# smrt-model/smrt

Hardware: AMD Instinct MI355X
Metric: snowpack x frequency DORT solves/sec (20 layers, 32 streams) (higher is better)
Workload: dtype f64

## Files before the change

include/smrt_dort.h:

```cpp
#ifndef SMRT_DORT_H
#define SMRT_DORT_H

#include <stdint.h>

#ifdef __cplusplus
extern "C" {
#endif
#if defined(__GNUC__)
#pragma GCC visibility push(default)
#endif

typedef struct smrt_dort_ctx smrt_dort_ctx;

#define SMRT_EM_IBA 0
#define SMRT_EM_DMRT_QCA_SHORTRANGE 1
#define SMRT_EM_DMRT_QCACP_SHORTRANGE 2
#define SMRT_EM_NONSCATTERING 3
#define SMRT_EM_HOST 4
#define SMRT_EM_IBA_INVERTED 5
#define SMRT_EM_IBA_HOST 6
#define SMRT_EM_RAYLEIGH_HOST 7
#define SMRT_MS_EXPONENTIAL 0
#define SMRT_MS_STICKY_HARD_SPHERES 1
#define SMRT_MS_INDEPENDENT_SPHERE 2
// ... 63 lines not shown
    int32_t host_interface_slots;
    const double* liquid_water;
    const double* host_iba_coeff;
} smrt_batch;

int32_t smrt_dort_out_stride(const smrt_batch* b);

int32_t smrt_dort_device_count(void);

int32_t smrt_dort_create(smrt_dort_ctx** ctx, int32_t device);
void smrt_dort_destroy(smrt_dort_ctx* ctx);
const char* smrt_dort_last_error(const smrt_dort_ctx* ctx);

int32_t smrt_dort_run(smrt_dort_ctx* ctx, const smrt_batch* batch, int64_t pair_begin, int64_t pair_count,
                      double* out, int32_t* status, double* layer_out, double* stream_out);

int32_t smrt_dort_run_pairs(smrt_dort_ctx* ctx, const smrt_batch* batch, const int64_t* pairs, int64_t n_pairs,
                            double* out, int32_t* status, double* layer_out, double* stream_out);

int32_t smrt_dort_upload(smrt_dort_ctx* ctx, const smrt_batch* batch, int64_t pair_begin, int64_t pair_count);
int32_t smrt_dort_upload_pairs(smrt_dort_ctx* ctx, const smrt_batch* batch, const int64_t* pairs, int64_t n_pairs);
int32_t smrt_dort_launch(smrt_dort_ctx* ctx, void* out_dev, void* status_dev);
int32_t smrt_dort_sync(smrt_dort_ctx* ctx);
int32_t smrt_dort_download(smrt_dort_ctx* ctx, double* out, int32_t* status, double* layer_out,
                           double* stream_out);

double smrt_dort_last_kernel_ms(smrt_dort_ctx* ctx);

int32_t smrt_dort_kernel_breakdown(smrt_dort_ctx* ctx, int32_t enable, double* ms3);

int32_t smrt_dort_set_diagonalisation(smrt_dort_ctx* ctx, int32_t mode);

enum { SMRT_INFO_PIPELINE = 0, SMRT_INFO_CHUNK_PAIRS, SMRT_INFO_CHUNKS, SMRT_INFO_PRUNE_ROUNDS, SMRT_INFO_STAGED_ITEMS,
       SMRT_INFO_BLOCK_THREADS, SMRT_INFO_N_MAX, SMRT_INFO_DIAGONALISATION, SMRT_INFO_RAYLEIGH_CLOSED_FORM, SMRT_INFO_COUNT };
enum { SMRT_DIAG_JACOBI = 0,
       SMRT_DIAG_SYMMETRIC = 1 };
enum { SMRT_PIPELINE_FUSED = 0,
       SMRT_PIPELINE_LDS_TWO_SLOT = 1,
       SMRT_PIPELINE_LDS_FOUR_SLOT = 2,
       SMRT_PIPELINE_LDS_REG = 3,
       SMRT_PIPELINE_FUSED_GMEM = 4,
       SMRT_PIPELINE_GMEM = 5,
       SMRT_PIPELINE_BIG = 6,
       SMRT_PIPELINE_GMEM_STRIP = 7,
       SMRT_PIPELINE_LDS_STRIP = 8 };
int32_t smrt_dort_launch_info(smrt_dort_ctx* ctx, int64_t* info, int32_t n);
double smrt_dort_total_kernel_ms(smrt_dort_ctx* ctx, int64_t* n_launches, int32_t reset);

int32_t smrt_dort_set_block_threads(smrt_dort_ctx* ctx, int32_t threads);

int32_t smrt_dort_set_pipeline(smrt_dort_ctx* ctx, int32_t split);

int32_t smrt_dort_finish_reg_lds_bytes(int32_t n_max_stream, int32_t n_layers_max);

int32_t smrt_dort_finish_strip_lds_bytes(int32_t n_max_stream, int32_t n_layers_max, int32_t wavefronts);

int32_t smrt_dort_jacobi_lds_bytes(int32_t n_max_stream, int32_t n_pol, int32_t size_class_columns);

double smrt_dort_sum_n3(smrt_dort_ctx* ctx);

int32_t smrt_dort_ft_even_phase(smrt_dort_ctx* ctx, int32_t emmodel, int32_t microstructure, double frequency,
                                double frac_volume, double temperature, double micro_p1, double micro_p2,
                                const double* mu_s, int32_t n_s, const double* mu_i, int32_t n_i, int32_t m_max,
                                int32_t npol, double* out);

int32_t smrt_dort_pair_cost(smrt_dort_ctx* ctx, double* cost);

// ... 200 lines not shown
```

smrt_amd/_native.py:

```python
from __future__ import annotations

import ctypes as C
import os
import threading

import numpy as np

from .core.error import SMRTError

_HERE = os.path.dirname(os.path.abspath(__file__))
LIB_PATH = os.environ.get("SMRT_DORT_LIB") or os.path.join(_HERE, "csrc", "libsmrt_dort.so")

EM_CODES = {"iba": 0, "dmrt_qca_shortrange": 1, "dmrt_qcacp_shortrange": 2, "nonscattering": 3, "host": 4,
            "iba_inverted": 5, "iba_host": 6, "rayleigh_host": 7}
MS_CODES = {"exponential": 0, "sticky_hard_spheres": 1, "independent_sphere": 2, "teubner_strey": 3,
            "unified_scaled_exponential": 0, "unified_sticky_hard_spheres": 1, "unified_teubner_strey": 3,
            "exponential_complex_k": 4, "sticky_hard_spheres_complex_k": 5, "independent_sphere_complex_k": 6,
            "teubner_strey_complex_k": 7}
SUBSTRATE_CODES = {"flat": 1, "reflector": 2, "host": 3}
NORM_CODES = {False: 0, None: 0, True: 1, "auto": 1, "forced": 2}
STATUS_MESSAGES = {
    1: "The eigen-decomposition did not converge in DORT.",
    2: "The re-normalization of the phase function exceeds the predefined threshold of 30%. This is likely because "
       "of a too large grain size or a bug in the phase function.",
# ... 1120 lines not shown
    def sar_sync(self):
        self._solver_call("smrt_sar_sync")

    def sar_download(self) -> SarOutput:
        return self._solver_download("sar", SarOutput)

    def sar_kernel_ms(self):
        return self._solver_kernel_ms("sar", 4)

    def ft_even_phase(self, emmodel, microstructure, frequency, frac_volume, temperature, p1, p2, mu_s, mu_i, m_max, npol):
        mu_s = np.ascontiguousarray(np.atleast_1d(mu_s), dtype=np.float64)
        mu_i = np.ascontiguousarray(np.atleast_1d(mu_i), dtype=np.float64)
        out = np.empty((npol, npol, m_max + 1, len(mu_s), len(mu_i)))
        with self.lock:
            self._check(self._lib.smrt_dort_ft_even_phase(
                self._h, EM_CODES[emmodel], MS_CODES[microstructure], float(frequency), float(frac_volume), float(temperature),
                float(p1), float(p2), _dptr(mu_s), len(mu_s), _dptr(mu_i), len(mu_i), int(m_max), int(npol), _dptr(out)),
                "smrt_dort_ft_even_phase")
        return out

    def pair_cost(self):
        _, pair_count = self._resident
        cost = np.empty(pair_count)
        self._check(self._lib.smrt_dort_pair_cost(self._h, _dptr(cost)), "smrt_dort_pair_cost")
        return cost

    PIPELINES = ("fused", "lds_two_slot", "lds_four_slot", "lds_reg", "fused_gmem", "gmem", "big", "gmem_strip", "lds_strip")

    def launch_info(self):
        v = (C.c_int64 * 16)()
        n = self._lib.smrt_dort_launch_info(self._h, v, 16)
        self._check(0 if n > 0 else -1, "smrt_dort_launch_info")
        keys = ("pipeline", "chunk_pairs", "chunks", "prune_rounds", "staged_items", "block_threads", "n_max", "diagonalisation",
                "rayleigh_closed_form")
        d = {k: int(v[i]) for i, k in enumerate(keys[:n])}
        d["pipeline"] = self.PIPELINES[d["pipeline"]]
        d["diagonalisation"] = self.DIAGONALISATIONS[d["diagonalisation"]]
        d["rayleigh_closed_form"] = bool(d.get("rayleigh_closed_form", 0))
        if d.get("staged_items", -1) < 0:
            d["staged_items"] = None
        return d

    @staticmethod
    def comm_library():
        lib = load_library()
        buf, version = C.create_string_buffer(1024), C.c_int32(0)
        if lib.smrt_dort_comm_library(buf, len(buf), C.byref(version)) != 0:
            raise SMRTError("RCCL is not available: " + buf.value.decode(errors="replace"))
        v = int(version.value)
        return buf.value.decode(), "%d.%d.%d" % (v // 10000, v // 100 % 100, v % 100) if v >= 10000 else str(v)

    @staticmethod
    def comm_unique_id():
        lib = load_library()
        buf = C.create_string_buffer(128)
        if lib.smrt_dort_comm_unique_id(buf) != 0:
            raise SMRTError("smrt_dort_comm_unique_id failed (is librccl available?)")
        return buf.raw

    def comm_init(self, world, rank, unique_id):
        self._check(self._lib.smrt_dort_comm_init(self._h, int(world), int(rank), bytes(unique_id)), "smrt_dort_comm_init")
        self.world, self.rank = int(world), int(rank)

    @staticmethod
    def comm_init_all(contexts):
        lib = load_library()
        arr = (C.c_void_p * len(contexts))(*[c._h for c in contexts])
        if lib.smrt_dort_comm_init_all(arr, len(contexts)) != 0:
            raise SMRTError("smrt_dort_comm_init_all failed: " + lib.smrt_dort_last_error(contexts[0]._h).decode())
        for r, c in enumerate(contexts):
            c.world, c.rank = len(contexts), r
# ... 81 lines not shown
```

smrt_amd/csrc/dort_ctx.hpp:

```cpp
#pragma once
#include <hip/hip_runtime.h>
#include <string>
#include <vector>

#include "dort_layout.hpp"

namespace smrt { struct PhaseRequest; struct FoBatch; }

struct DevBuf {
    void* p = nullptr;
    size_t cap = 0;
    hipError_t reserve(size_t bytes) {
        if (bytes <= cap) return hipSuccess;
        if (p) (void)hipFree(p);
        p = nullptr;
        cap = 0;
        hipError_t e = hipMalloc(&p, bytes);
        if (e == hipSuccess) cap = bytes;
        return e;
    }
    void release() { if (p) (void)hipFree(p); p = nullptr; cap = 0; }
};

struct smrt_dort_ctx {
// ... 6 lines not shown
    bool uploaded = false;
    int out_stride = 0;
    int nt = 256;
    size_t lds_bytes = 0;
    size_t prep_lds_bytes = 0;
    size_t finish2_lds_bytes = 0;
    size_t finish_reg_lds_bytes = 0;
    size_t prep_wide_lds_bytes = 0;
    bool prep_wide = false;
    size_t finish_strip_lds_bytes = 0, finish_strip4_lds_bytes = 0;
    bool finish_strip4 = false;
    bool finish_strip = false;
    bool finish_reg = false;
    int finish_mode = -1;
    bool finish2 = true;
    float last_ms = 0.f;
    double total_ms = 0.0;
    int64_t n_launch = 0;
    bool timing_pending = false;
    bool breakdown_on = false;
    std::vector<hipEvent_t> bd_events;
    std::vector<int> bd_kind;
    size_t bd_used = 0;
    int max_lds = 0;
    bool split = true;
    long long chunk_pairs = 0;
    int lanes = 1;
    hipStream_t lane_stream[4] = {nullptr, nullptr, nullptr, nullptr};
    hipEvent_t lane_ev[4] = {nullptr, nullptr, nullptr, nullptr};
    hipEvent_t fork_ev = nullptr;
    size_t jacobi_lds = 0;
    int diag_mode = -1;
    bool eig = false;
    size_t jacobi16_lds = 0;
    smrt::DevStage stage{};
    bool gmem_path = false;
    bool gmem_split = false;
    bool big = false;
    int jac_in_lds = 0;
    bool active = false;
    int gmem_grid = 0;
    long long ws_stride = 0;
    int nmax_rows = 0;
    void* comm = nullptr;
    int comm_world = 0, comm_rank = 0;
    DevBuf d_gather_out, d_gather_status, d_scalar;
    struct FirstOrderState* first_order = nullptr;
    struct SuccessiveOrderState* successive_order = nullptr;
    struct SuccessiveOrderActiveState* successive_order_active = nullptr;
    struct MultiFresnelState* multifresnel = nullptr;
    struct SecondOrderState* second_order = nullptr;
    struct LrmState* lrm = nullptr;
    struct SarState* sar = nullptr;
};

#ifndef SMRT_JACOBI_NT
#define SMRT_JACOBI_NT 256
#endif

namespace smrt_launch {
hipError_t prep(smrt_dort_ctx* ctx, const smrt::DevBatch& c, int nt);
hipError_t prep_wide(smrt_dort_ctx* ctx, const smrt::DevBatch& c);
hipError_t finish(smrt_dort_ctx* ctx, const smrt::DevBatch& c, int nt, bool two_slot);
void occupancy_report(smrt_dort_ctx* ctx, int nt);
hipError_t finish_reg(smrt_dort_ctx* ctx, const smrt::DevBatch& c);
hipError_t finish_strip(smrt_dort_ctx* ctx, const smrt::DevBatch& c);
// ... 26 lines not shown
```

smrt_amd/csrc/dort_dense.hpp:

```cpp
#pragma once
#include "spmd.hpp"
#include <math.h>
#include <string.h>
#include "dort_physics.hpp"

namespace smrt {

struct Tile2D { int rmask, cshift, cols_per_wave; };
SMRT_DEV Tile2D make_tile(int R) {
    Tile2D t;
    int sh = 6;
    if (R <= 32) sh = 5;
    if (R <= 16) sh = 4;
    if (R <= 8) sh = 3;
    if (R <= 4) sh = 2;
    t.rmask = (1 << sh) - 1; t.cshift = sh; t.cols_per_wave = SMRT_LANES >> sh;
    return t;
}
template <int NT, class Body>
SMRT_DEV void for_2d(int R, int C, Body body) {
    const int t = tid();
    const int lane = t & (SMRT_LANES - 1), wave = t / SMRT_LANES;
    constexpr int NW = NT / SMRT_LANES;
    const Tile2D tl = make_tile(R);
// ... 288 lines not shown
    const int lane = tid() & (SMRT_LANES - 1), lr = lane & 15, lk = lane >> 4;
    const int col = tj * 16 + lr;
#pragma unroll
    for (int reg = 0; reg < 4; ++reg) {
        const int row = ti * 16 + lk + 4 * reg;
        if (row < N && col < N) f(reg, row, col);
    }
}

template <int NT, bool PK = false>
SMRT_DEV void lt_times_l_mfma(const double* Lp, const double* Lm, double* C, int N, int LD, bool reverse_cols = false) {
    const int wave = tid() / SMRT_LANES;
    constexpr int NW = NT / SMRT_LANES;
    const int RT = (N + 15) >> 4;
    for (int tix = wave; tix < RT * RT; tix += NW) {
        const int ti = tix % RT, tj = tix / RT;
        double c[4] = {0.0, 0.0, 0.0, 0.0};
        const int kmin = 16 * (ti > tj ? ti : tj);
        const int lane = tid() & (SMRT_LANES - 1), lr = lane & 15, lk = lane >> 4;
        const int i = ti * 16 + lr, j = tj * 16 + lr;
        const int ic = i < N ? i : N - 1, jc = j < N ? j : N - 1;
        const int abase = sidx<PK>(ic, ic, LD) - ic, bbase = sidx<PK>(jc, jc, LD) - jc;
        for (int k0 = kmin; k0 < N; k0 += 4) {
            const int k = k0 + lk, kc = k < N ? k : N - 1;
            const double av = Lp[abase + (kc > ic ? kc : ic)], bv = Lm[bbase + (kc > jc ? kc : jc)];
            const bool kin = k < N;
            mfma_f64_16x16x4((kin && k >= i) ? av : 0.0, (kin && k >= j) ? bv : 0.0, c);
        }
        tile_foreach(ti, tj, N, [&](int reg, int row, int col) { C[(reverse_cols ? N - 1 - col : col) * LD + row] = c[reg]; });
    }
    block_sync();
}

template <int NT>
SMRT_DEV void l_times_m_mfma(const double* Lp, const double* Bm, double* C, int N, int LD) {
    const int wave = tid() / SMRT_LANES;
    constexpr int NW = NT / SMRT_LANES;
    constexpr int TPW = 3;
    const int RT = (N + 15) >> 4;
    const int NG = (RT + TPW - 1) / TPW;
    const int lane = tid() & (SMRT_LANES - 1), lr = lane & 15, lk = lane >> 4;
    for (int u = wave; u < RT * NG; u += NW) {
        const int ti = u % RT, tg = u / RT;
        double c[TPW][4];
#pragma unroll
        for (int q = 0; q < TPW; ++q)
#pragma unroll
            for (int reg = 0; reg < 4; ++reg) c[q][reg] = 0.0;
        const int i = ti * 16 + lr, ic = i < N ? i : N - 1;
        const int kend = (ti * 16 + 16 < N) ? ti * 16 + 16 : N;
        const int nq = (RT - tg * TPW < TPW) ? RT - tg * TPW : TPW;
        for (int k0 = 0; k0 < kend; k0 += 16) {
            double av[4], bv[TPW][4];
#pragma unroll
            for (int kk = 0; kk < 4; ++kk) {
                const int k = k0 + 4 * kk + lk, kc = k < N ? k : N - 1;
                const double x = Lp[kc * LD + ic];
                av[kk] = (i < N && k <= i && k < N) ? x : 0.0;
#pragma unroll
                for (int q = 0; q < TPW; ++q) {
                    bv[q][kk] = 0.0;
                    if (q < nq) {
                        const int j = (tg * TPW + q) * 16 + lr, jc = j < N ? j : N - 1;
                        const double y = Bm[jc * LD + kc];
                        bv[q][kk] = (j < N && k < N) ? y : 0.0;
                    }
// ... 824 lines not shown
```

smrt_amd/csrc/dort_hip.hip:

```cpp
#include <hip/hip_runtime.h>
#include <algorithm>
#include <cstddef>
#include <cstdio>
#include <cstdlib>
#include <cstring>
#include <string>
#include <vector>

#include "dort_ctx.hpp"
#include "dort_eig_kernel.hpp"
#include "dort_rayleigh_kernel.hpp"
#include "dort_jacobi_big.hpp"
#include "dort_host_common.hpp"
#include "dort_phase_kernel.hpp"
#include "dort_finish_reg.hpp"
#include "dort_finish_strip.hpp"
#include "solver_host.hpp"

using namespace smrt;

static int upload_array(smrt_dort_ctx* ctx, DevBuf& buf, const void* src, size_t bytes) {
    HIPCHK(buf.reserve(bytes));
    HIPCHK(hipMemcpyAsync(buf.p, src, bytes, hipMemcpyHostToDevice, ctx->stream));
    return 0;
}


static DevBatch chunk_of(const smrt_dort_ctx* ctx, const DevBatch& d, long long c0, long long cn) {
    DevBatch c = d;
    c.pair_begin = d.pair_begin + c0; c.pair_count = cn;
    c.out = d.out + c0 * ctx->out_stride; c.status = d.status + c0;
    c.layer_out = d.layer_out + c0 * (long long)d.Lmax * 5;
    c.stream_out = d.stream_out + c0 * (long long)(1 + d.n_max_stream);
    c.n3_out = d.n3_out + c0; c.stage_out = d.stage_out + c0 * 16;
    if (d.dispatch) c.dispatch = d.dispatch + c0;
    return c;
}

#ifndef SMRT_DORT_LANES_DEFAULT
#define SMRT_DORT_LANES_DEFAULT 1
#endif
#ifndef SMRT_FINISH_STRIP_DEFAULT
#define SMRT_FINISH_STRIP_DEFAULT 1
#endif
#ifndef SMRT_FINISH_REG_DEFAULT
#define SMRT_FINISH_REG_DEFAULT 1
#endif
static hipError_t launch_pipeline(smrt_dort_ctx* ctx, const DevBatch& d) {
    const long long items_per_pair = (long long)(ctx->active ? d.m_max + 1 : 1) * d.Lmax;
    const long long modes = ctx->active ? d.m_max + 1 : 1;
    if (getenv("SMRT_DORT_DEBUG_OCCUPANCY") && !ctx->gmem_path && !ctx->active) smrt_launch::occupancy_report(ctx, ctx->nt);
    const int rounds = (d.prune_tau > 0.0 && !d.coherent && getenv("SMRT_DORT_NO_PRUNE_ROUNDS") == nullptr) ? std::min(4, d.Lmax) : 1;
    auto prep = [&](const DevBatch& c, unsigned grid) {
        if (ctx->big) return smrt_launch::prep_gmem_big(ctx, c, grid, ctx->active, ctx->nmax_rows <= 256 ? 4 : 6);
        if (ctx->prep_wide) return smrt_launch::prep_wide(ctx, c);
        if (ctx->gmem_split) return smrt_launch::prep_gmem(ctx, c, grid, ctx->active);
        return ctx->active ? smrt_launch::active_prep(ctx, c, ctx->nt) : smrt_launch::prep(ctx, c, ctx->nt);
    };
    auto finish = [&](const DevBatch& c, unsigned grid) {
        if (ctx->big) return smrt_launch::finish_gmem_big(ctx, c, grid, ctx->active, ctx->nmax_rows <= 256 ? 4 : 6);
        if (ctx->finish_strip) return smrt_launch::finish_strip(ctx, c);
        if (ctx->gmem_split) return smrt_launch::finish_gmem(ctx, c, grid, ctx->active);
        if (ctx->finish_strip4) return smrt_launch::finish_strip4(ctx, c);
        if (ctx->finish_reg) return smrt_launch::finish_reg(ctx, c);
        return ctx->active ? smrt_launch::active_finish(ctx, c, ctx->nt) : smrt_launch::finish(ctx, c, ctx->nt, ctx->finish2);
    };
    const hipStream_t main_stream = ctx->stream;
    const DevStage stage0 = ctx->stage;
    const int lanes = (ctx->lanes > 1 && d.pair_count > ctx->chunk_pairs) ? ctx->lanes : 1;
    struct Restore { smrt_dort_ctx* c; hipStream_t s; DevStage st; ~Restore() { c->stream = s; c->stage = st; } } restore{ctx, main_stream, stage0};
    if (lanes > 1) {
        hipError_t e;
        if ((e = hipEventRecord(ctx->fork_ev, main_stream)) != hipSuccess) return e;
        for (int k = 0; k < lanes; ++k)
            if ((e = hipStreamWaitEvent(ctx->lane_stream[k], ctx->fork_ev, 0)) != hipSuccess) return e;
    }
    auto timed = [&](int kind, auto&& launch) -> hipError_t {
        if (!ctx->breakdown_on) return launch();
        for (int k = 0; k < 2; ++k)
            if (ctx->bd_used + k >= ctx->bd_events.size()) {
                hipEvent_t ev;
                hipError_t e = hipEventCreate(&ev);
                if (e != hipSuccess) return e;
                ctx->bd_events.push_back(ev);
            }
        hipError_t e = hipEventRecord(ctx->bd_events[ctx->bd_used], ctx->stream);
        if (e != hipSuccess) return e;
        e = launch();
        if (e != hipSuccess) return e;
        e = hipEventRecord(ctx->bd_events[ctx->bd_used + 1], ctx->stream);
        ctx->bd_used += 2;
        ctx->bd_kind.push_back(kind);
        return e;
    };
    if (ctx->breakdown_on) { ctx->bd_used = 0; ctx->bd_kind.clear(); }
    long long chunk_index = 0;
    for (long long c0 = 0; c0 < d.pair_count; c0 += ctx->chunk_pairs, ++chunk_index) {
        const long long cn = std::min<long long>(ctx->chunk_pairs, d.pair_count - c0);
        DevBatch c = chunk_of(ctx, d, c0, cn);
        const unsigned grid = (unsigned)(ctx->gmem_path ? std::min<long long>(cn, ctx->gmem_grid) : cn);
// ... 200 lines not shown
    ctx->eig = false;
    int big_min = 128;
    if (const char* e = getenv("SMRT_DORT_BIG_MIN_N")) big_min = std::max(64, atoi(e));
    ctx->big = ctx->gmem_path && ctx->split && plan.NMAX > big_min && getenv("SMRT_DORT_NO_BIG_PIPELINE") == nullptr &&
               (size_t)make_jacobi_big_plan(b->n_max_stream, P).total * sizeof(double) <= (size_t)ctx->max_lds;
    const bool split128 = ctx->gmem_path && ctx->split && !ctx->big && plan.NMAX <= 128 &&
        (size_t)make_jacobi_plan(b->n_max_stream, P).total * sizeof(double) <= (size_t)ctx->max_lds &&
        (size_t)make_plan(b->n_max_stream, P, b->n_layers_max, b->n_theta, nphi, 0, actd_fin, 0, 2).total * sizeof(double) <= (size_t)ctx->max_lds &&
        (size_t)make_plan(b->n_max_stream, P, b->n_layers_max, b->n_theta, nphi, 0, actd, 1).total * sizeof(double) <= (size_t)ctx->max_lds;
    if (split128) ctx->jac_in_lds = 1;
    ctx->gmem_split = ctx->big || split128;
    if (ctx->big) ctx->jac_in_lds = 0;
    if ((!ctx->gmem_path && ctx->split) || ctx->gmem_split) {
        const size_t nmodes = ctx->active ? (size_t)b->m_max + 1 : 1;
        const size_t mat = (size_t)plan.NMAX * plan.LD;
        const int linv_stride = (plan.NMAX > 64) ? 2048 : 1024;
        const size_t per_pair = nmodes * b->n_layers_max * ((2 * mat + 2 * plan.NMAX + linv_stride) * sizeof(double) + sizeof(int));
        double budget = 12.0e9;
        if (ctx->big) {
            size_t free_b = 0, total_b = 0;
            if (hipMemGetInfo(&free_b, &total_b) == hipSuccess) budget = std::max(budget, 0.6 * (double)(free_b + ctx->d_stL.cap + ctx->d_stB.cap));
        }
        const bool one_per_cu = ctx->gmem_split && !ctx->big;
        if (one_per_cu) budget = 40.0e9;
        long long chunk = (long long)(budget / (double)per_pair);
        if (chunk < 1) chunk = 1;
        if (one_per_cu && chunk >= 512) chunk -= chunk % 256;
        const long long chunk_cap = chunk;
        if (chunk > pair_count) chunk = pair_count;
        {
            int want = ctx->diag_mode < 0 ? SMRT_DIAG_SYMMETRIC : ctx->diag_mode;
            if (const char* e = getenv("SMRT_DORT_EIG")) want = atoi(e) ? SMRT_DIAG_SYMMETRIC : SMRT_DIAG_JACOBI;
            ctx->eig = !ctx->gmem_path && !ctx->active && plan.NMAX <= 64 && want == SMRT_DIAG_SYMMETRIC;
        }
        ctx->lanes = 1;
        if (!ctx->gmem_path) {
            int want = ctx->eig ? 3 : SMRT_DORT_LANES_DEFAULT;
            if (const char* e = getenv("SMRT_DORT_LANES")) want = atoi(e);
            ctx->lanes = std::max(1, std::min(4, want));
            while (ctx->lanes > 1 && pair_count < 1024LL * ctx->lanes) --ctx->lanes;
        }
        {
            long long nchunks = (pair_count + chunk - 1) / chunk;
            if (ctx->lanes > 1) nchunks = ((nchunks + ctx->lanes - 1) / ctx->lanes) * ctx->lanes;
            chunk = (pair_count + nchunks - 1) / nchunks;
            if (one_per_cu && nchunks > 1) chunk = std::min(chunk_cap, ((chunk + 255) / 256) * 256);
        }
        ctx->chunk_pairs = chunk;
        for (int k = 0; k < ctx->lanes && ctx->lanes > 1; ++k) {
            if (!ctx->lane_stream[k]) HIPCHK(hipStreamCreateWithFlags(&ctx->lane_stream[k], hipStreamNonBlocking));
            if (!ctx->lane_ev[k]) HIPCHK(hipEventCreateWithFlags(&ctx->lane_ev[k], hipEventDisableTiming));
        }
        if (ctx->lanes > 1 && !ctx->fork_ev) HIPCHK(hipEventCreateWithFlags(&ctx->fork_ev, hipEventDisableTiming));
        const size_t items = (size_t)chunk * ctx->lanes * b->n_layers_max * nmodes;
        HIPCHK(ctx->d_stL.reserve(items * mat * sizeof(double)));
        HIPCHK(ctx->d_stB.reserve(items * mat * sizeof(double)));
        HIPCHK(ctx->d_std.reserve(items * plan.NMAX * sizeof(double)));
        HIPCHK(ctx->d_sts.reserve(items * plan.NMAX * sizeof(double)));
        HIPCHK(ctx->d_stn.reserve(items * sizeof(int)));
        HIPCHK(ctx->d_sti.reserve(ctx->big ? 8 : items * linv_stride * sizeof(double)));
        ctx->stage.L = (double*)ctx->d_stL.p; ctx->stage.B = (double*)ctx->d_stB.p;
        ctx->stage.d = (double*)ctx->d_std.p; ctx->stage.sigma = (double*)ctx->d_sts.p;
        ctx->stage.n = (int*)ctx->d_stn.p; ctx->stage.Linv = ctx->big ? nullptr : (double*)ctx->d_sti.p;
        ctx->stage.linv_stride = linv_stride;
        ctx->stage.mat_stride = (long long)mat; ctx->stage.vec_stride = plan.NMAX;
        {
// ... 292 lines not shown

int32_t smrt_dort_launch_info(smrt_dort_ctx* ctx, int64_t* info, int32_t n) {
    if (!ctx || !info || n < 0) return -1;
    if (!ctx->uploaded) { ctx->err = "no batch uploaded"; return -1; }
    const DevBatch& d = ctx->dev;
    const bool lds_pipeline = !ctx->gmem_path && ctx->split && ctx->chunk_pairs > 0 && (!ctx->active || ctx->finish2);
    int64_t v[SMRT_INFO_COUNT] = {0};
    v[SMRT_INFO_PIPELINE] = ctx->gmem_split ? (ctx->big ? SMRT_PIPELINE_BIG : ctx->finish_strip ? SMRT_PIPELINE_GMEM_STRIP : SMRT_PIPELINE_GMEM)
                          : lds_pipeline ? (ctx->finish_strip4 ? SMRT_PIPELINE_LDS_STRIP : ctx->finish_reg ? SMRT_PIPELINE_LDS_REG : ctx->finish2 ? SMRT_PIPELINE_LDS_TWO_SLOT : SMRT_PIPELINE_LDS_FOUR_SLOT)
                          : ctx->gmem_path ? SMRT_PIPELINE_FUSED_GMEM : SMRT_PIPELINE_FUSED;
    const bool three = ctx->gmem_split || lds_pipeline;
    v[SMRT_INFO_CHUNK_PAIRS] = three ? ctx->chunk_pairs : d.pair_count;
    v[SMRT_INFO_CHUNKS] = three ? (d.pair_count + ctx->chunk_pairs - 1) / ctx->chunk_pairs : 1;
    const int rounds = (three && d.prune_tau > 0.0 && !d.coherent && getenv("SMRT_DORT_NO_PRUNE_ROUNDS") == nullptr) ? std::min(4, d.Lmax) : 1;
    v[SMRT_INFO_PRUNE_ROUNDS] = rounds;
    v[SMRT_INFO_STAGED_ITEMS] = -1;
    if (three && (rounds > 1 || d.coherent) && ctx->n_launch + (ctx->timing_pending ? 1 : 0) > 0) {
        HIPCHK(hipSetDevice(ctx->device));
        HIPCHK(hipStreamSynchronize(ctx->stream));
        const long long items_per_pair = (long long)(ctx->active ? d.m_max + 1 : 1) * d.Lmax;
        const long long last = d.pair_count - (v[SMRT_INFO_CHUNKS] - 1) * ctx->chunk_pairs;
        std::vector<int> h((size_t)(last * items_per_pair));
        const int lanes = (ctx->lanes > 1 && d.pair_count > ctx->chunk_pairs) ? ctx->lanes : 1;
        const long long lane = (v[SMRT_INFO_CHUNKS] - 1) % lanes;
        HIPCHK(hipMemcpy(h.data(), ctx->stage.n + lane * ctx->chunk_pairs * items_per_pair, sizeof(int) * h.size(), hipMemcpyDeviceToHost));
        long long staged = 0;
        for (int x : h) staged += (x > 0);
        v[SMRT_INFO_STAGED_ITEMS] = staged;
    }
    v[SMRT_INFO_BLOCK_THREADS] = ctx->nt;
    v[SMRT_INFO_N_MAX] = ctx->nmax_rows;
    v[SMRT_INFO_DIAGONALISATION] = (three && ctx->eig) ? SMRT_DIAG_SYMMETRIC : SMRT_DIAG_JACOBI;
    v[SMRT_INFO_RAYLEIGH_CLOSED_FORM] = (three && d.rayleigh_direct) ? 1 : 0;
    for (int k = 0; k < n && k < SMRT_INFO_COUNT; ++k) info[k] = v[k];
    return SMRT_INFO_COUNT;
}

double smrt_dort_total_kernel_ms(smrt_dort_ctx* ctx, int64_t* n_launches, int32_t reset) {
    if (!ctx) return -1.0;
    const double tot = ctx->total_ms;
    if (n_launches) *n_launches = ctx->n_launch;
    if (reset) { ctx->total_ms = 0.0; ctx->n_launch = 0; }
    return tot;
}

int32_t smrt_dort_download(smrt_dort_ctx* ctx, double* out, int32_t* status, double* layer_out, double* stream_out) {
    if (!ctx) return -1;
    if (!ctx->uploaded) { ctx->err = "no batch uploaded"; return -1; }
    HIPCHK(hipSetDevice(ctx->device));
    const DevBatch& d = ctx->dev;
    const size_t np = (size_t)d.pair_count;
    if (out) HIPCHK(hipMemcpyAsync(out, d.out, sizeof(double) * np * ctx->out_stride, hipMemcpyDeviceToHost, ctx->stream));
    if (status) HIPCHK(hipMemcpyAsync(status, d.status, sizeof(int32_t) * np, hipMemcpyDeviceToHost, ctx->stream));
    if (layer_out) HIPCHK(hipMemcpyAsync(layer_out, d.layer_out, sizeof(double) * np * d.Lmax * 5, hipMemcpyDeviceToHost, ctx->stream));
    if (stream_out) HIPCHK(hipMemcpyAsync(stream_out, d.stream_out, sizeof(double) * np * (1 + d.n_max_stream), hipMemcpyDeviceToHost, ctx->stream));
    return smrt_dort_sync(ctx);
}

double smrt_dort_sum_n3(smrt_dort_ctx* ctx) {
    if (!ctx || !ctx->uploaded) return -1.0;
    if (hipSetDevice(ctx->device) != hipSuccess) return -1.0;
    std::vector<double> h((size_t)ctx->dev.pair_count);
    if (hipMemcpy(h.data(), ctx->dev.n3_out, sizeof(double) * h.size(), hipMemcpyDeviceToHost) != hipSuccess) return -1.0;
    double s = 0.0;
    for (double v : h) s += v;
    return s;
// ... 76 lines not shown
```

smrt_amd/csrc/dort_layout.hpp:

```cpp
#pragma once
#include "spmd.hpp"
#include <math.h>
#include <string.h>

#if defined(SMRT_HOST_EMU)
#define SMRT_HD_EARLY inline
#else
#define SMRT_HD_EARLY __host__ __device__ inline
#endif

namespace smrt {

struct DevBatch {
    int S, Lmax, F, n_theta;
    int emmodel, micro, mode, n_max_stream, m_max, normalization, rayleigh_jeans;
    int want_layer_out, want_stream_out;
    int jac_in_lds;
    long long pair_begin, pair_count;
    const long long* pair_map;
    const int* n_layers;
    const double* thickness;
    const double* frac_volume;
    const double* temperature;
    const double* p1;
// ... 18 lines not shown
    int sub_kind;
    const double *sub_p1, *sub_p2;
    const double* sub_T;
    const double *atm_down, *atm_up, *atm_trans;
    double phi;
    double jacobi_skip2, jacobi_exit2;
    double prune_tau;
    int layer_lo, layer_hi;
    const int* pair_done;
    const int* dispatch;
    double* out;
    int* status;
    double* layer_out;
    double* stream_out;
    double* n3_out;
    double* stage_out;
    int rayleigh_direct;
};

struct DevStage {
    double* L;
    double* B;
    double* d;
    double* sigma;
    int* n;
    long long mat_stride;
    int vec_stride;
    double* Linv;
    double* ws;
    int linv_stride;
    double* eig_e;
    double* eig_rot;
    long long rot_stride;
};

constexpr int kStageDirect = 4096;
SMRT_DEV int stage_rows(int n) { return n > 0 ? (n & (kStageDirect - 1)) : n; }
SMRT_DEV bool stage_direct(int n) { return n > kStageDirect; }

SMRT_DEV long long global_pair(const DevBatch& b, long long p) {
    return b.pair_map ? b.pair_map[b.pair_begin + p] : b.pair_begin + p;
}

SMRT_DEV long long dispatched_pair(const DevBatch& b, long long w) { return b.dispatch ? (long long)b.dispatch[w] : w; }

SMRT_DEV long long jacobi_item_of_block(const DevBatch& b, long long blk) {
    const int span = b.layer_hi - b.layer_lo;
    long long row = blk / span;
    if (b.dispatch) {
        const int nmodes = (b.mode == 1) ? b.m_max + 1 : 1;
        row = (long long)b.dispatch[row / nmodes] * nmodes + row % nmodes;
    }
    return row * b.Lmax + b.layer_lo + (blk % span);
}

constexpr double kCSpeed = 299792458.0;
constexpr double kPlanck = 6.62607015e-34;
constexpr double kBoltzmann = 1.380649e-23;
constexpr double kFreezing = 273.15;
constexpr double kPi = 3.14159265358979323846;

enum { EM_IBA = 0, EM_DMRT = 1, EM_QCACP = 2, EM_NONSCAT = 3, EM_HOST = 4, EM_IBA_INV = 5, EM_IBA_HOST = 6, EM_RAYLEIGH_HOST = 7 };
SMRT_HD_EARLY bool em_has_rayleigh_phase(int em) { return em == EM_DMRT || em == EM_QCACP || em == EM_NONSCAT || em == EM_RAYLEIGH_HOST; }
enum { MS_EXP = 0, MS_SHS = 1, MS_SPHERE = 2, MS_TS = 3, MS_EXPC = 4, MS_SHSC = 5, MS_SPHEREC = 6, MS_TSC = 7 };
enum { ST_OK = 0, ST_EIGEN = 1, ST_NORM = 2, ST_ALBEDO = 3, ST_SINGULAR = 4, ST_INPUT = 5, ST_COHERENT = 6 };
enum { SUB_NONE = 0, SUB_FLAT = 1, SUB_REFLECTOR = 2, SUB_HOST = 3 };
// ... 126 lines not shown
```

smrt_amd/csrc/dort_passive.hpp:

```cpp
#pragma once
#include "spmd.hpp"
#include <math.h>
#include <string.h>
#include "dort_gauss_jordan.hpp"
#include "dort_interface_dense.hpp"

namespace smrt {

template <int NT>
SMRT_DEV int pruned_layer_count(const DevStage& stg, long long item0, int L, const double* thick, double* tau,
                                double limit) {
    const int t = tid();
    const int lane = t % SMRT_LANES, wave = t / SMRT_LANES;
    constexpr int NW = NT / SMRT_LANES;
    for (int l = wave; l < L; l += NW) {
        const long long item = item0 + l;
        const int N = stage_rows(stg.n[item]);
        double m = 1e300;
        for (int r = lane; r < N; r += SMRT_LANES) {
            const double sg = stg.sigma[item * stg.vec_stride + r];
            m = sg < m ? sg : m;
        }
        for (int k = 1; k < SMRT_LANES; k <<= 1) { const double o = shfl_xor(m, k); m = o < m ? o : m; }
        if (lane == 0) tau[l] = (N > 0) ? m * thick[l] : -1.0;
// ... 460 lines not shown
            s.d[r] = uu / s.wrow[r];
        }
        block_sync();
        if (s.ints[0] != ST_OK) {
            if (MODE == 1) { layer_failed(l, s.ints[0]); continue; }
            fail_pair<NT>(b, p, s.ints[0], out_stride); return;
        }
        if (ray_direct) {
            const long long item = p * (long long)b.Lmax + l;
            double* gI = stg->Linv + item * stg->linv_stride;
            for (int r = t; r < N; r += NT) { gI[2 + n + r] = s.u[r]; stg->d[item * stg->vec_stride + r] = s.d[r]; }
            for (int j = t; j < n; j += NT) gI[2 + j] = s.mu[j];
            if (t == 0) { gI[0] = ke; gI[1] = s.pa[l]; stg->n[item] = N + kStageDirect; }
            block_sync();
            continue;
        }
        for_2d<NT>(N, N, [&](int r, int c) {
            if (r >= c) {
                const double uu = 0.5 * s.u[r] * s.u[c];
                const double dg = (r == c) ? ke / s.mrow[r] : 0.0;
                s.M0[sidx<PK>(r, c, LD)] = dg - uu * s.M0[sidx<PK>(r, c, LD)];
                s.M1[sidx<PK>(r, c, LD)] = dg - uu * s.M1[sidx<PK>(r, c, LD)];
            }
        });
        block_sync();
        SMRT_STAGE(SG_CHOL);
        if (!(dense_mfma ? chol2_mfma<NT, PK>(s.M0, s.M1, dense_scratch, &s.ints[2], N, LD,
                                       (MODE == 1 && CH <= 2 && stg->Linv) ? stg->Linv + (p * (long long)b.Lmax + l) * stg->linv_stride : nullptr)
                      : chol2<NT>(s.M0, s.M1, N, LD))) {
            if (MODE == 1) { layer_failed(l, ST_ALBEDO); continue; }
            fail_pair<NT>(b, p, ST_ALBEDO, out_stride); return;
        }
        SMRT_STAGE(SG_BTL);
        if (MODE == 1) {
            lt_times_l_mfma<NT, PK>(s.M0, s.M1, stg->B + (p * (long long)b.Lmax + l) * stg->mat_stride, N, LD,
#ifdef SMRT_NO_COLUMN_REVERSAL
                                false);
#else
                                true);
#endif
        } else {
        if (dense_mfma) lt_times_l_mfma<NT>(s.M0, s.M1, s.M2, N, LD);
        else lt_times_l<NT>(s.M0, s.M1, s.M2, N, LD);
        }
        }
        if (MODE == 1) {
            const long long item = p * (long long)b.Lmax + l;
            double* gL = stg->L + item * stg->mat_stride;
            for_2d<NT>(N, N, [&](int r, int c) { gL[c * LD + r] = (PK && r < c) ? 0.0 : s.M0[sidx<PK>(r, c, LD)]; });
            for (int r = t; r < N; r += NT) stg->d[item * stg->vec_stride + r] = s.d[r];
            if (t == 0) stg->n[item] = N;
            block_sync();
            continue;
        }
        SMRT_STAGE(SG_JACOBI);
        if (MODE == 0) {
            double* Jm = (plan.o_jac >= 0) ? lds_base + plan.o_jac : s.M2;
            if (Jm != s.M2) { for_2d<NT>(N, N, [&](int r, int c) { Jm[c * LD + r] = s.M2[c * LD + r]; }); block_sync(); }
            if (!jacobi_onesided<NT, JW, GS, RPL>(Jm, N, LD, s.sigma, s.rsig, &s.ints[1], &n_sweeps, s.sub_acc)) {
                fail_pair<NT>(b, p, ST_EIGEN, out_stride); return;
            }
            if (Jm != s.M2) { for_2d<NT>(N, N, [&](int r, int c) { s.M2[c * LD + r] = Jm[c * LD + r]; }); block_sync(); }
        } else {
            const long long item = p * (long long)b.Lmax + l;
            const double* gL = stg->L + item * stg->mat_stride;
            const double* gB = stg->B + item * stg->mat_stride;
// ... 182 lines not shown
```

smrt_amd/csrc/k_eig.hip:

```cpp
#include <cstdlib>
#include "dort_ctx.hpp"
#include "dort_device.hpp"
#include "dort_eig_kernel.hpp"

using namespace smrt;

#define SMRT_EIG_ROWS(NP_, CALL) \
    if constexpr (LO < (NP_) && (NP_) - 8 < HI) if (rows <= (NP_)) { CALL; return; }
#define SMRT_EIG_ROWS16(NP_, CALL) \
    if constexpr (LO < (NP_) && (NP_) - 16 < HI) if (rows <= (NP_)) { CALL; return; }

template <int LO, int HI>
__global__ __launch_bounds__(64) void dort_eig_gram_kernel(DevBatch b, DevStage st) {
    const long long item = uniform(jacobi_item_of_block(b, (long long)blockIdx.x));
    const int rows = uniform(eig_item_rows(b, st, item));
    if (rows <= LO || rows > HI) return;
    SMRT_EIG_ROWS16(16, (eig_gram_item<16>(st, item))) SMRT_EIG_ROWS16(32, (eig_gram_item<32>(st, item)))
    SMRT_EIG_ROWS16(48, (eig_gram_item<48>(st, item))) SMRT_EIG_ROWS16(64, (eig_gram_item<64>(st, item)))
}

template <int LO, int HI>
__global__ __launch_bounds__(64) void dort_eig_tridiag_kernel(DevBatch b, DevStage st) {
    const long long item = uniform(jacobi_item_of_block(b, (long long)blockIdx.x));
    const int rows = uniform(eig_item_rows(b, st, item));
// ... 16 lines not shown
    SMRT_EIG_ROWS(56, (eig_vectors_item<56>(st, item, ring))) SMRT_EIG_ROWS(64, (eig_vectors_item<64>(st, item, ring)))
}

__global__ __launch_bounds__(kEigChaseLanes) void dort_eig_chase_kernel(DevBatch b, DevStage st, long long items) {
    extern __shared__ __attribute__((aligned(16))) double smrt_lds[];
    const long long blk = (long long)blockIdx.x * kEigChaseLanes + threadIdx.x;
    if (blk >= items) return;
    const long long item = jacobi_item_of_block(b, blk);
    if (eig_item_rows(b, st, item) <= 0) return;
    const int nmax = st.vec_stride;
    eig_chase_lane(st, item, smrt_lds + threadIdx.x, smrt_lds + kEigChaseLanes * nmax + threadIdx.x);
}

namespace smrt_launch {
template <int LO, int HI>
static hipError_t go_gram(smrt_dort_ctx* ctx, const DevBatch& c, long long items) {
    hipLaunchKernelGGL((dort_eig_gram_kernel<LO, HI>), dim3((unsigned)items), dim3(64), 0, ctx->stream, c, ctx->stage);
    return hipGetLastError();
}
template <int LO, int HI>
static hipError_t go_tridiag(smrt_dort_ctx* ctx, const DevBatch& c, long long items) {
    hipLaunchKernelGGL((dort_eig_tridiag_kernel<LO, HI>), dim3((unsigned)items), dim3(64), 0, ctx->stream, c, ctx->stage);
    return hipGetLastError();
}
template <int LO, int HI>
static hipError_t go_vectors(smrt_dort_ctx* ctx, const DevBatch& c, long long items) {
    hipLaunchKernelGGL((dort_eig_vectors_kernel<LO, HI>), dim3((unsigned)items), dim3(64), 0, ctx->stream, c, ctx->stage);
    return hipGetLastError();
}

hipError_t eig(smrt_dort_ctx* ctx, const DevBatch& c, long long items) {
    const int nmax = ctx->nmax_rows;
    hipError_t e;
    if ((e = go_gram<0, 32>(ctx, c, items)) != hipSuccess) return e;
    if (nmax > 32 && (e = go_gram<32, 48>(ctx, c, items)) != hipSuccess) return e;
    if (nmax > 48 && (e = go_gram<48, 64>(ctx, c, items)) != hipSuccess) return e;
    if ((e = go_tridiag<0, 32>(ctx, c, items)) != hipSuccess) return e;
    if (nmax > 32 && (e = go_tridiag<32, 48>(ctx, c, items)) != hipSuccess) return e;
    if (nmax > 48 && (e = go_tridiag<48, 64>(ctx, c, items)) != hipSuccess) return e;
    {
        const size_t lds = (size_t)2 * kEigChaseLanes * nmax * sizeof(double);
        e = hipFuncSetAttribute((const void*)dort_eig_chase_kernel, hipFuncAttributeMaxDynamicSharedMemorySize, (int)lds);
        if (e != hipSuccess) return e;
        hipLaunchKernelGGL(dort_eig_chase_kernel, dim3((unsigned)((items + kEigChaseLanes - 1) / kEigChaseLanes)), dim3(kEigChaseLanes), lds, ctx->stream, c, ctx->stage, items);
        if ((e = hipGetLastError()) != hipSuccess) return e;
    }
    if ((e = go_vectors<0, 32>(ctx, c, items)) != hipSuccess) return e;
    if (nmax > 32 && (e = go_vectors<32, 48>(ctx, c, items)) != hipSuccess) return e;
    if (nmax > 48 && (e = go_vectors<48, 64>(ctx, c, items)) != hipSuccess) return e;
    return hipSuccess;
}
}
```

Before: 177,900.

## Fuse Gram matrix computation into prep kernel for symmetric eigen path

When the symmetric eigen path is active with 256-thread blocks, the prep kernel now writes L, d and n to staging, computes the L^T L product, and then forms the Gram matrix in place with MFMA tiles. The separate eig gram kernel launches are skipped in that case. This is meant to remove extra kernel launches and a global-memory round trip of the intermediate matrix. The cost is more work and more register pressure in the prep kernel, and the behaviour can be switched off through an environment variable.

```diff
diff --git a/include/smrt_dort.h b/include/smrt_dort.h
--- a/include/smrt_dort.h
+++ b/include/smrt_dort.h
@@ -119,7 +119,8 @@
 int32_t smrt_dort_set_diagonalisation(smrt_dort_ctx* ctx, int32_t mode);
 
 enum { SMRT_INFO_PIPELINE = 0, SMRT_INFO_CHUNK_PAIRS, SMRT_INFO_CHUNKS, SMRT_INFO_PRUNE_ROUNDS, SMRT_INFO_STAGED_ITEMS,
-       SMRT_INFO_BLOCK_THREADS, SMRT_INFO_N_MAX, SMRT_INFO_DIAGONALISATION, SMRT_INFO_RAYLEIGH_CLOSED_FORM, SMRT_INFO_COUNT };
+       SMRT_INFO_BLOCK_THREADS, SMRT_INFO_N_MAX, SMRT_INFO_DIAGONALISATION, SMRT_INFO_RAYLEIGH_CLOSED_FORM, SMRT_INFO_GRAM_IN_PREP,
+       SMRT_INFO_COUNT };
 enum { SMRT_DIAG_JACOBI = 0,
        SMRT_DIAG_SYMMETRIC = 1 };
 enum { SMRT_PIPELINE_FUSED = 0,
diff --git a/smrt_amd/_native.py b/smrt_amd/_native.py
--- a/smrt_amd/_native.py
+++ b/smrt_amd/_native.py
@@ -1176,11 +1176,12 @@
         n = self._lib.smrt_dort_launch_info(self._h, v, 16)
         self._check(0 if n > 0 else -1, "smrt_dort_launch_info")
         keys = ("pipeline", "chunk_pairs", "chunks", "prune_rounds", "staged_items", "block_threads", "n_max", "diagonalisation",
-                "rayleigh_closed_form")
+                "rayleigh_closed_form", "gram_in_prep")
         d = {k: int(v[i]) for i, k in enumerate(keys[:n])}
         d["pipeline"] = self.PIPELINES[d["pipeline"]]
         d["diagonalisation"] = self.DIAGONALISATIONS[d["diagonalisation"]]
         d["rayleigh_closed_form"] = bool(d.get("rayleigh_closed_form", 0))
+        d["gram_in_prep"] = bool(d.get("gram_in_prep", 0))
         if d.get("staged_items", -1) < 0:
             d["staged_items"] = None
         return d
diff --git a/smrt_amd/csrc/dort_ctx.hpp b/smrt_amd/csrc/dort_ctx.hpp
--- a/smrt_amd/csrc/dort_ctx.hpp
+++ b/smrt_amd/csrc/dort_ctx.hpp
@@ -62,6 +62,7 @@
     size_t jacobi_lds = 0;
     int diag_mode = -1;
     bool eig = false;
+    bool prep_gram = false;
     size_t jacobi16_lds = 0;
     smrt::DevStage stage{};
     bool gmem_path = false;
diff --git a/smrt_amd/csrc/dort_dense.hpp b/smrt_amd/csrc/dort_dense.hpp
--- a/smrt_amd/csrc/dort_dense.hpp
+++ b/smrt_amd/csrc/dort_dense.hpp
@@ -344,6 +344,91 @@
     block_sync();
 }
 
+template <int G>
+SMRT_DEV void gram_tiles_mfma(const double* Bl, double* gS, int N, int LD, int first, int stride, int ntl) {
+    const int lane = tid() & (SMRT_LANES - 1), lr = lane & 15, lk = lane >> 4;
+    int ti[G], tj[G], rac[G], rbc[G];
+    bool ain[G], bin[G];
+    tile4 acc[G];
+#pragma unroll
+    for (int g = 0; g < G; ++g) {
+        const int idx = first + g * stride < ntl ? first + g * stride : 0;
+        int r = 0;
+        while ((r + 1) * (r + 2) / 2 <= idx) ++r;
+        ti[g] = r; tj[g] = idx - r * (r + 1) / 2;
+        const int ra = 16 * ti[g] + lr, rb = 16 * tj[g] + lr;
+        ain[g] = ra < N; bin[g] = rb < N;
+        rac[g] = ain[g] ? ra : N - 1; rbc[g] = bin[g] ? rb : N - 1;
+        acc[g] = tile_zero();
+    }
+    const int kend = (N + 3) & ~3;
+    for (int k0 = 0; k0 < kend; k0 += 4) {
+        const int col = k0 + lk, cc = col < N ? col : N - 1;
+        double av[G], bv[G];
+#pragma unroll
+        for (int g = 0; g < G; ++g) { av[g] = Bl[cc * LD + rac[g]]; bv[g] = Bl[cc * LD + rbc[g]]; }
+#pragma unroll
+        for (int g = 0; g < G; ++g) mfma_tile((col < N && ain[g]) ? av[g] : 0.0, (col < N && bin[g]) ? bv[g] : 0.0, acc[g]);
+    }
+#pragma unroll
+    for (int g = 0; g < G; ++g) {
+        if (first + g * stride >= ntl) continue;
+#pragma unroll
+        for (int reg = 0; reg < 4; ++reg) {
+            const int row = 16 * ti[g] + lk + 4 * reg, col = 16 * tj[g] + lr;
+            if (row < N && col < N) {
+                gS[col * LD + row] = acc[g][reg];
+                if (ti[g] != tj[g]) gS[row * LD + col] = acc[g][reg];
+            }
+        }
+    }
+}
+
+template <int NT>
+SMRT_DEV void lt_times_l_gram_mfma(double* Lp, const double* Lm, double* gS, int N, int LD, bool reverse_cols) {
+    constexpr int NW = NT / SMRT_LANES;
+    constexpr int TPW = (16 + NW - 1) / NW;
+    const int wave = tid() / SMRT_LANES;
+    const int lane = tid() & (SMRT_LANES - 1), lr = lane & 15, lk = lane >> 4;
+    const int RT = (N + 15) >> 4;
+    double c[TPW][4];
+#pragma unroll
+    for (int q = 0; q < TPW; ++q) {
+        c[q][0] = c[q][1] = c[q][2] = c[q][3] = 0.0;
+        const int tix = wave + q * NW;
+        if (tix < RT * RT) {
+            const int ti = tix % RT, tj = tix / RT;
+            const int kmin = 16 * (ti > tj ? ti : tj);
+            const int i = ti * 16 + lr, j = tj * 16 + lr;
+            const int ic = i < N ? i : N - 1, jc = j < N ? j : N - 1;
+            const int abase = sidx<true>(ic, ic, LD) - ic, bbase = sidx<true>(jc, jc, LD) - jc;
+            for (int k0 = kmin; k0 < N; k0 += 4) {
+                const int k = k0 + lk, kc = k < N ? k : N - 1;
+                const double av = Lp[abase + (kc > ic ? kc : ic)], bv = Lm[bbase + (kc > jc ? kc : jc)];
+                const bool kin = k < N;
+                mfma_f64_16x16x4((kin && k >= i) ? av : 0.0, (kin && k >= j) ? bv : 0.0, c[q]);
+            }
+        }
+    }
+    block_sync();
+    double* Bl = Lp;
+#pragma unroll
+    for (int q = 0; q < TPW; ++q) {
+        const int tix = wave + q * NW;
+        if (tix < RT * RT)
+            tile_foreach(tix % RT, tix / RT, N, [&](int reg, int row, int col) { Bl[(reverse_cols ? N - 1 - col : col) * LD + row] = c[q][reg]; });
+    }
+    block_sync();
+    constexpr int GT = (10 + NW - 1) / NW;
+    const int ntl = RT * (RT + 1) / 2;
+    const int mine = wave < ntl ? (ntl - wave + NW - 1) / NW : 0;
+    if (GT >= 3 && mine >= 3) {
+        for (int first = wave; first < ntl; first += 3 * NW) gram_tiles_mfma<3>(Bl, gS, N, LD, first, NW, ntl);
+    } else if (GT >= 2 && mine == 2) gram_tiles_mfma<2>(Bl, gS, N, LD, wave, NW, ntl);
+    else if (mine == 1) gram_tiles_mfma<1>(Bl, gS, N, LD, wave, NW, ntl);
+    block_sync();
+}
+
 template <int NT>
 SMRT_DEV void l_times_m_mfma(const double* Lp, const double* Bm, double* C, int N, int LD) {
     const int wave = tid() / SMRT_LANES;
diff --git a/smrt_amd/csrc/dort_hip.hip b/smrt_amd/csrc/dort_hip.hip
--- a/smrt_amd/csrc/dort_hip.hip
+++ b/smrt_amd/csrc/dort_hip.hip
@@ -46,6 +46,8 @@
 #ifndef SMRT_FINISH_REG_DEFAULT
 #define SMRT_FINISH_REG_DEFAULT 1
 #endif
+static bool gram_in_prep(const smrt_dort_ctx* ctx) { return ctx->eig && ctx->prep_gram && ctx->nt == 256; }
+
 static hipError_t launch_pipeline(smrt_dort_ctx* ctx, const DevBatch& d) {
     const long long items_per_pair = (long long)(ctx->active ? d.m_max + 1 : 1) * d.Lmax;
     const long long modes = ctx->active ? d.m_max + 1 : 1;
@@ -66,6 +68,7 @@
         return ctx->active ? smrt_launch::active_finish(ctx, c, ctx->nt) : smrt_launch::finish(ctx, c, ctx->nt, ctx->finish2);
     };
     const hipStream_t main_stream = ctx->stream;
+    ctx->stage.gram_in_prep = gram_in_prep(ctx) ? 1 : 0;
     const DevStage stage0 = ctx->stage;
     const int lanes = (ctx->lanes > 1 && d.pair_count > ctx->chunk_pairs) ? ctx->lanes : 1;
     struct Restore { smrt_dort_ctx* c; hipStream_t s; DevStage st; ~Restore() { c->stream = s; c->stage = st; } } restore{ctx, main_stream, stage0};
@@ -332,6 +335,8 @@
             int want = ctx->diag_mode < 0 ? SMRT_DIAG_SYMMETRIC : ctx->diag_mode;
             if (const char* e = getenv("SMRT_DORT_EIG")) want = atoi(e) ? SMRT_DIAG_SYMMETRIC : SMRT_DIAG_JACOBI;
             ctx->eig = !ctx->gmem_path && !ctx->active && plan.NMAX <= 64 && want == SMRT_DIAG_SYMMETRIC;
+            const char* g = getenv("SMRT_DORT_PREP_GRAM");
+            ctx->prep_gram = ctx->eig && !(g && atoi(g) == 0);
         }
         ctx->lanes = 1;
         if (!ctx->gmem_path) {
@@ -690,6 +695,7 @@
     v[SMRT_INFO_N_MAX] = ctx->nmax_rows;
     v[SMRT_INFO_DIAGONALISATION] = (three && ctx->eig) ? SMRT_DIAG_SYMMETRIC : SMRT_DIAG_JACOBI;
     v[SMRT_INFO_RAYLEIGH_CLOSED_FORM] = (three && d.rayleigh_direct) ? 1 : 0;
+    v[SMRT_INFO_GRAM_IN_PREP] = (three && gram_in_prep(ctx)) ? 1 : 0;
     for (int k = 0; k < n && k < SMRT_INFO_COUNT; ++k) info[k] = v[k];
     return SMRT_INFO_COUNT;
 }
diff --git a/smrt_amd/csrc/dort_layout.hpp b/smrt_amd/csrc/dort_layout.hpp
--- a/smrt_amd/csrc/dort_layout.hpp
+++ b/smrt_amd/csrc/dort_layout.hpp
@@ -74,6 +74,7 @@
     double* eig_e;
     double* eig_rot;
     long long rot_stride;
+    int gram_in_prep;
 };
 
 constexpr int kStageDirect = 4096;
diff --git a/smrt_amd/csrc/dort_passive.hpp b/smrt_amd/csrc/dort_passive.hpp
--- a/smrt_amd/csrc/dort_passive.hpp
+++ b/smrt_amd/csrc/dort_passive.hpp
@@ -516,6 +516,22 @@
             fail_pair<NT>(b, p, ST_ALBEDO, out_stride); return;
         }
         SMRT_STAGE(SG_BTL);
+        if constexpr (PK && NT == 256) {
+            if (stg->gram_in_prep) {
+                const long long item = p * (long long)b.Lmax + l;
+                double* gL = stg->L + item * stg->mat_stride;
+                for_2d<NT>(N, N, [&](int r, int c) { gL[c * LD + r] = (r < c) ? 0.0 : s.M0[sidx<PK>(r, c, LD)]; });
+                for (int r = t; r < N; r += NT) stg->d[item * stg->vec_stride + r] = s.d[r];
+                if (t == 0) stg->n[item] = N;
+                lt_times_l_gram_mfma<NT>(s.M0, s.M1, stg->B + item * stg->mat_stride, N, LD,
+#ifdef SMRT_NO_COLUMN_REVERSAL
+                                         false);
+#else
+                                         true);
+#endif
+                continue;
+            }
+        }
         if (MODE == 1) {
             lt_times_l_mfma<NT, PK>(s.M0, s.M1, stg->B + (p * (long long)b.Lmax + l) * stg->mat_stride, N, LD,
 #ifdef SMRT_NO_COLUMN_REVERSAL
diff --git a/smrt_amd/csrc/k_eig.hip b/smrt_amd/csrc/k_eig.hip
--- a/smrt_amd/csrc/k_eig.hip
+++ b/smrt_amd/csrc/k_eig.hip
@@ -72,9 +72,11 @@
 hipError_t eig(smrt_dort_ctx* ctx, const DevBatch& c, long long items) {
     const int nmax = ctx->nmax_rows;
     hipError_t e;
-    if ((e = go_gram<0, 32>(ctx, c, items)) != hipSuccess) return e;
-    if (nmax > 32 && (e = go_gram<32, 48>(ctx, c, items)) != hipSuccess) return e;
-    if (nmax > 48 && (e = go_gram<48, 64>(ctx, c, items)) != hipSuccess) return e;
+    if (!ctx->stage.gram_in_prep) {
+        if ((e = go_gram<0, 32>(ctx, c, items)) != hipSuccess) return e;
+        if (nmax > 32 && (e = go_gram<32, 48>(ctx, c, items)) != hipSuccess) return e;
+        if (nmax > 48 && (e = go_gram<48, 64>(ctx, c, items)) != hipSuccess) return e;
+    }
     if ((e = go_tridiag<0, 32>(ctx, c, items)) != hipSuccess) return e;
     if (nmax > 32 && (e = go_tridiag<32, 48>(ctx, c, items)) != hipSuccess) return e;
     if (nmax > 48 && (e = go_tridiag<48, 64>(ctx, c, items)) != hipSuccess) return e;
```

Result: no change. 179,100 (median of 6 runs) (+0.7%).
